# espnet/espnet

Hardware: AMD Instinct MI355X
Metric: audio-seconds/sec (RTF^-1), Conformer-ASR, 10 s utterances (higher is better)
Workload: dtype bf16; 1 GPU; BASELINE.json configs[1]: Conformer-small (12x256d, 4 heads), HIP STFT/log-mel + HIP encoder + greedy CTC (G1) + hypotheses collated to the host, 32 x 10 s utterances per GPU per step, V=5000; batch_per_gpu=32, global_batch=32, parallelism=utterance-dp1

## Files before the change

### espnet_amd/csrc/block.hip

```cpp
#include <stdio.h>
#include <stdlib.h>

#include <type_traits>

#include "em_common.h"
#include "switches.h"

namespace {

constexpr int D = 256;
constexpr int BM = 32;
constexpr int NT = 256;
constexpr int NC = 256;
constexpr int UNIT = 32768;
constexpr int PAR_FLOATS = EM_BLOCK_PARAM_GROUP;
constexpr int PAR_BYTES = PAR_FLOATS * 4;
constexpr int MAX_GROUPS = 4;
constexpr int PAR_OFF = 0;
constexpr int RED_OFF = PAR_OFF + MAX_GROUPS * PAR_BYTES;
constexpr int TOUCH_OFF = RED_OFF + 2048;
constexpr int TILE_OFF = TOUCH_OFF + 1024;
constexpr int ABUF_OFF = TILE_OFF + 32768;
constexpr int WK_OFF = ABUF_OFF + 16384;
constexpr int XCH_OFF = WK_OFF + 32768;
constexpr int XSLOT = 8192;
constexpr int SMEM_BYTES = XCH_OFF + 49152;
static_assert(ABUF_OFF % 1024 == 0 && TILE_OFF % 1024 == 0 && SMEM_BYTES <= 160 * 1024, "LDS layout");
constexpr int KW_MAX = 31, TROWS_MAX = BM + KW_MAX - 1;
constexpr int TPITCH = 528;
static_assert(TROWS_MAX * TPITCH <= 32768, "conv tile");
constexpr int CPAR_OFF = XCH_OFF;
constexpr int ABUF64_OFF = XCH_OFF + 8192;
static_assert(PAR_BYTES <= 8192 && ABUF64_OFF + 32768 <= SMEM_BYTES, "fold layout");

typedef const __attribute__((address_space(1))) unsigned char* GU8;
typedef const __attribute__((address_space(1))) bf16x8* GFRAG;
constexpr int BAR_UNIT = 1, BAR_PARAMS = 2, BAR_TILE = 4, BAR_LAST = 8;

#ifndef EM_BLOCK_DBG
#define EM_BLOCK_DBG 0
#endif

#ifndef EM_BLOCK_VAR
#define EM_BLOCK_VAR 0
#endif
#ifndef EM_BLOCK_FINE
#define EM_BLOCK_FINE 0
#endif

#define EM_LGKM0() asm volatile("s_waitcnt lgkmcnt(0)" ::: "memory")

__device__ __forceinline__ const unsigned char* em_uniform_ptr(const unsigned char* p) {
  const unsigned long long v = (unsigned long long)p;
  const unsigned lo = __builtin_amdgcn_readfirstlane((unsigned)v);
  const unsigned hi = __builtin_amdgcn_readfirstlane((unsigned)(v >> 32));
  return (const unsigned char*)(((unsigned long long)hi << 32) | lo);
}

template <int N, typename F>
__device__ __forceinline__ void em_static_for(F&& f) {
  if constexpr (N > 0) {
    em_static_for<N - 1>(f);
    f(std::integral_constant<int, N - 1>{});
  }
}

template <int MODE, int KWT = 31, bool RELU = false>
__global__ __launch_bounds__(NT, 1) void block_kernel(const EmBlockArgs a_in, long long* __restrict__ stamps) {
  const EmBlockArgs& a = a_in;
  const void *ffm_w1 = a_in.ffm_w1, *ffm_w2 = a_in.ffm_w2, *ff_w1 = a_in.ff_w1, *ff_w2 = a_in.ff_w2;
  const float *ffm_b1g = a_in.ffm_b1g, *ff_b1g = a_in.ff_b1g;
  int nsplit = 1;
  if constexpr (RELU && (MODE & (EM_BLOCK_A | EM_BLOCK_D | EM_BLOCK_T)) != 0) {
    nsplit = a_in.ffn_split > 1 ? a_in.ffn_split : 1;
    if (nsplit > 1) {
      const int nch_all = ((a_in.ff >> 6) + 1) & ~1, nch_s = nch_all / nsplit, sidx = blockIdx.z;
      const size_t wo = (size_t)sidx * nch_s * UNIT;
      if (ffm_w1) { ffm_w1 = (const unsigned char*)ffm_w1 + wo; ffm_w2 = (const unsigned char*)ffm_w2 + wo; }
      if (ff_w1) { ff_w1 = (const unsigned char*)ff_w1 + wo; ff_w2 = (const unsigned char*)ff_w2 + wo; }
      if (ffm_b1g) ffm_b1g += sidx * nch_s * 64;
      if (ff_b1g) ff_b1g += sidx * nch_s * 64;
    }
  }
  bool ffn_exit = false;
  constexpr int KW = KWT, HALF = KWT / 2, TROWS = BM + KWT - 1;
  static_assert(KWT == 31 || KWT == 15, "depthwise conv width");
  constexpr int dbg = EM_BLOCK_DBG;
  using MM = Mma<bf16>;
  constexpr bool HAS_C = (MODE & EM_BLOCK_C) != 0, HAS_D = (MODE & EM_BLOCK_D) != 0;
  constexpr bool HAS_A = (MODE & EM_BLOCK_A) != 0, FINAL = (MODE & EM_BLOCK_FINAL) != 0;
  constexpr bool CTC = (MODE & EM_BLOCK_CTC) != 0;
  constexpr bool FOLD = HAS_C && HAS_D;
  constexpr bool ATT = (MODE & EM_BLOCK_ATT) != 0;
  constexpr bool HAS_T = (MODE & EM_BLOCK_T) != 0, HAS_Q = (MODE & EM_BLOCK_Q) != 0;
  static_assert(!(HAS_T || HAS_Q) || (RELU && !HAS_C && !HAS_D && !HAS_A && !FINAL && !CTC && ATT == HAS_T), "block<ATT|T>, block<Q>, block<ATT|T|Q>");
  static_assert(!ATT || ((HAS_C != HAS_T) && !HAS_D && !HAS_A && !FINAL), "block<ATT|C> and block<ATT|T..> are the instantiations with the attention phase");
  static_assert(!FOLD || KWT == 31, "the folded C part is written for the 15-frame halo of k = 31");
  extern __shared__ __attribute__((aligned(1024))) unsigned char smem[];
  unsigned char* const abuf = smem + ABUF_OFF;
  float* const red0 = (float*)(smem + RED_OFF);
  float* const par = (float*)(smem + PAR_OFF);

  const int tid = threadIdx.x, lane = tid & 63;
  const int wave = __builtin_amdgcn_readfirstlane(tid >> 6);
  const int nf = wave & 3;
  const int lr = lane & 15, lg = lane >> 4;
  int b = blockIdx.y, t0 = blockIdx.x * BM;
  const int T = a.T;
  if constexpr (ATT) {
    const int gx = gridDim.x, lid = blockIdx.y * gx + blockIdx.x, grp = lid / (8 * gx);
    if ((int)blockIdx.y < a.B && grp * 8 + 8 <= a.B) {
      b = grp * 8 + (lid & 7);
      t0 = ((lid - grp * 8 * gx) >> 3) * BM;
    }
  }

  bool row_ok[2];
  size_t mrow[2];
#pragma unroll
  for (int mi = 0; mi < 2; ++mi) {
    const int t = t0 + mi * 16 + lr;
    row_ok[mi] = t < T;
    mrow[mi] = (size_t)b * T + (t < T ? t : T - 1);
  }
  const int ncol = nf * 16 + lg * 4;
  const int swz = lr & 7;
  const int tile_wr = lr * 128 + (((2 * nf + (lg >> 1)) ^ swz) << 4) + (lg & 1) * 8;
  const int nch = (((a.ff >> 6) + 1) & ~1) / nsplit;
  int nts = 0;
  auto stamp = [&](int code) __attribute__((always_inline)) {
    if constexpr (EM_BLOCK_FINE) {
      if (stamps && blockIdx.x == (gridDim.x > 3 ? 3 : 0) && blockIdx.y == (a.B > 5 ? 5 : 0) && blockIdx.z == 0 && lane == 0 && nts < 64)
        stamps[wave * 64 + nts] = ((long long)code << 56) | ((long long)__builtin_amdgcn_s_memtime() & 0xffffffffffffffll);
    } else {
      if (stamps && blockIdx.x == 0 && blockIdx.y == 0 && blockIdx.z < 4 && tid == 0 && nts < 64)
        stamps[blockIdx.z * 64 + nts] = ((long long)code << 56) | ((long long)__builtin_amdgcn_s_memtime() & 0xffffffffffffffll);
    }
    ++nts;
  };
  auto fstamp = [&](int code) __attribute__((always_inline)) {
    if constexpr (EM_BLOCK_FINE) stamp(code);
  };
  auto rstamp = [&](int code) __attribute__((always_inline)) {
    if constexpr (EM_BLOCK_FINE || RELU) stamp(code);
  };
  stamp(1);
  int nbar = 0;
  auto bar = [&](int code) __attribute__((always_inline)) {
    (void)code;
    ++nbar;
    EM_LGKM0();
    __builtin_amdgcn_s_barrier();
  };

  float4 xr[2][4];
  bf16x8 act[2][8];
  auto load_x = [&]() __attribute__((always_inline)) {
#pragma unroll
    for (int mi = 0; mi < 2; ++mi)
#pragma unroll
      for (int f = 0; f < 4; ++f) xr[mi][f] = *(const float4*)(a.x + mrow[mi] * D + 64 * f + ncol);
  };
  float* const xdst = FOLD ? a.x_out : a.x;
  auto store_x = [&]() __attribute__((always_inline)) {
#pragma unroll
    for (int mi = 0; mi < 2; ++mi)
      if (row_ok[mi]) {
#pragma unroll
        for (int f = 0; f < 4; ++f) *(float4*)(xdst + mrow[mi] * D + 64 * f + ncol) = xr[mi][f];
      }
  };
  constexpr bool PLAIN = !RELU && !FOLD;
  constexpr bool X_EARLY_A = PLAIN && HAS_A && !(EM_BLOCK_VAR & 0x10000);
  constexpr bool X_EARLY_C = PLAIN && HAS_C && !(EM_BLOCK_VAR & 0x20000);
  constexpr bool GLU_COUNTED = PLAIN && HAS_C && (EM_BLOCK_VAR & 0x40000) != 0;
  typedef __attribute__((ext_vector_type(2))) unsigned su32x2;
  typedef __attribute__((ext_vector_type(4))) unsigned su32x4;
  constexpr unsigned ROW_MASKED = 0x80000000u;
  unsigned rowoff[2];
#pragma unroll
  for (int mi = 0; mi < 2; ++mi) rowoff[mi] = row_ok[mi] ? (unsigned)(t0 + mi * 16 + lr) * (D * 4u) + ncol * 4u : ROW_MASKED;
  auto rows_rsrc = [&](const void* base, int esz) __attribute__((always_inline)) {
    const unsigned char* p = em_uniform_ptr((const unsigned char*)base + (size_t)b * T * D * esz);
    return __builtin_amdgcn_make_buffer_rsrc(const_cast<unsigned char*>(p), 0, T * D * esz, 0x00020000);
  };
  auto put_f32x4 = [&](__amdgpu_buffer_rsrc_t rs, int mi, int f, const float4& v) __attribute__((always_inline)) {
    __builtin_amdgcn_raw_buffer_store_b128(__builtin_bit_cast(su32x4, v), rs, rowoff[mi] + 256 * f, 0, 0);
  };
  auto put_bf16x4 = [&](__amdgpu_buffer_rsrc_t rs, int mi, int f, const bf16x4& v) __attribute__((always_inline)) {
    __builtin_amdgcn_raw_buffer_store_b64(__builtin_bit_cast(su32x2, v), rs, (rowoff[mi] >> 1) + 128 * f, 0, 0);
  };
  auto store_x_counted = [&]() __attribute__((always_inline)) {
    const __amdgpu_buffer_rsrc_t rs = rows_rsrc(xdst, 4);
#pragma unroll
    for (int mi = 0; mi < 2; ++mi)
#pragma unroll
      for (int f = 0; f < 4; ++f) put_f32x4(rs, mi, f, xr[mi][f]);
  };
  auto load_act = [&]() __attribute__((always_inline)) {
#pragma unroll
    for (int mi = 0; mi < 2; ++mi)
#pragma unroll
      for (int ks = 0; ks < 8; ++ks)
        act[mi][ks] = *(const bf16x8*)(abuf + ((ks >> 1) * 32 + mi * 16 + lr) * 128 + ((((ks & 1) * 4 + lg) ^ swz) << 4));
  };
  int nln = 0;
  auto ln_partials = [&](const float4 (&v)[2][4], float* red) {
#pragma unroll
    for (int mi = 0; mi < 2; ++mi) {
      float s = 0.f;
#pragma unroll
      for (int f = 0; f < 4; ++f) s += (v[mi][f].x + v[mi][f].y) + (v[mi][f].z + v[mi][f].w);
      const float m0 = s * (1.0f / 16.0f);
      float q = 0.f;
#pragma unroll
      for (int f = 0; f < 4; ++f) {
        const float dx = v[mi][f].x - m0, dy = v[mi][f].y - m0, dz = v[mi][f].z - m0, dw = v[mi][f].w - m0;
        q += (dx * dx + dy * dy) + (dz * dz + dw * dw);
      }
      {
        const Pair2 ps = wave_xor16_pair(s), pq = wave_xor16_pair(q);
        q = pq.a + pq.b + (ps.a - ps.b) * (ps.a - ps.b) * (1.0f / 32.0f);
        s = ps.a + ps.b;
      }
      {
        const Pair2 ps = wave_xor32_pair(s), pq = wave_xor32_pair(q);
        q = pq.a + pq.b + (ps.a - ps.b) * (ps.a - ps.b) * (1.0f / 64.0f);
        s = ps.a + ps.b;
      }
      red[nf * 32 + mi * 16 + lr] = s;
      red[128 + nf * 32 + mi * 16 + lr] = q;
    }
  };
  auto ln_finish = [&](const float* red, float mean[2], float rstd[2]) __attribute__((always_inline)) {
#pragma unroll
    for (int mi = 0; mi < 2; ++mi) {
      const int m = mi * 16 + lr;
      const float s0 = red[m], s1 = red[32 + m], s2 = red[64 + m], s3 = red[96 + m];
      const float q0 = red[128 + m], q1 = red[160 + m], q2 = red[192 + m], q3 = red[224 + m];
      const float sa = s0 + s1, sb = s2 + s3;
      const float qa = q0 + q1 + (s0 - s1) * (s0 - s1) * (1.0f / 128.0f);
      const float qb = q2 + q3 + (s2 - s3) * (s2 - s3) * (1.0f / 128.0f);
      const float qq = qa + qb + (sa - sb) * (sa - sb) * (1.0f / 256.0f);
      mean[mi] = (sa + sb) * (1.0f / D);
      const float var = qq * (1.0f / D) + a.eps;
      const float y0 = __builtin_amdgcn_rsqf(var);
      rstd[mi] = y0 * (1.5f - 0.5f * var * y0 * y0);
    }
  };
  auto no_pre = [] {};
  auto ln_stats = [&](float mean[2], float rstd[2], int code, auto&& pre1, auto n1c) __attribute__((always_inline)) {
    constexpr int N1 = decltype(n1c)::value;
    float* const red = red0 + (nln & 1) * 256;
    ++nln;
    pre1();
    ln_partials(xr, red);
    if constexpr (N1 > 0 && !(EM_BLOCK_VAR & 32)) {
#pragma unroll
      for (int i = 0; i < N1; ++i) {
        __builtin_amdgcn_sched_group_barrier(0x020, 1, 0);
        __builtin_amdgcn_sched_group_barrier(0x002, N1 > 16 ? 4 : 7, 0);
      }
    }
    fstamp(11);
    bar(code);
    fstamp(12);
    ln_finish(red, mean, rstd);
  };
  auto ln_apply_pre = [&](const float* pb, int go, int bo, float4 y[2][4], int code, auto&& pre1, auto n1c) __attribute__((always_inline)) {
    float mean[2], rstd[2];
    ln_stats(mean, rstd, code, pre1, n1c);
#pragma unroll
    for (int f = 0; f < 4; ++f) {
      const float4 g4 = *(const float4*)(pb + go + 64 * f + ncol);
      const float4 b4 = *(const float4*)(pb + bo + 64 * f + ncol);
#pragma unroll
      for (int mi = 0; mi < 2; ++mi) {
        y[mi][f].x = (xr[mi][f].x - mean[mi]) * rstd[mi] * g4.x + b4.x;
        y[mi][f].y = (xr[mi][f].y - mean[mi]) * rstd[mi] * g4.y + b4.y;
        y[mi][f].z = (xr[mi][f].z - mean[mi]) * rstd[mi] * g4.z + b4.z;
        y[mi][f].w = (xr[mi][f].w - mean[mi]) * rstd[mi] * g4.w + b4.w;
      }
    }
  };
  auto ln_apply = [&](const float* pb, int go, int bo, float4 y[2][4], int code) __attribute__((always_inline)) {
    ln_apply_pre(pb, go, bo, y, code, no_pre, std::integral_constant<int, 0>{});
  };
  auto ln_to_act_pre = [&](const float* pb, int go, int bo, int code, auto&& pre1, auto n1c, auto&& pre2, auto n2c) __attribute__((always_inline)) {
    constexpr int N2 = decltype(n2c)::value;
    float4 y[2][4];
    __builtin_amdgcn_sched_barrier(0);
    ln_apply_pre(pb, go, bo, y, 0, pre1, n1c);
    pre2();
#pragma unroll
    for (int mi = 0; mi < 2; ++mi)
#pragma unroll
      for (int f = 0; f < 4; ++f) {
        bf16x4 pk = {(bf16)y[mi][f].x, (bf16)y[mi][f].y, (bf16)y[mi][f].z, (bf16)y[mi][f].w};
        *(bf16x4*)(abuf + f * 4096 + mi * 2048 + tile_wr) = pk;
      }
    if constexpr (N2 > 0 && !(EM_BLOCK_VAR & 32)) {
#pragma unroll
      for (int i = 0; i < N2; ++i) {
        __builtin_amdgcn_sched_group_barrier(0x020, 1, 0);
        __builtin_amdgcn_sched_group_barrier(0x002, N2 > 8 ? 6 : 10, 0);
      }
    }
    fstamp(13);
    bar(code);
    fstamp(14);
    load_act();
  };
  auto ln_to_act = [&](const float* pb, int go, int bo, int code) __attribute__((always_inline)) {
    ln_to_act_pre(pb, go, bo, code, no_pre, std::integral_constant<int, 0>{}, no_pre, std::integral_constant<int, 0>{});
  };
  struct WF {
    bf16x8 v[8];
  };
  WF ring[4];
  const unsigned voff = nf * 8192 + lane * 16;
  auto read_unit = [&](const void* base, int u, WF& w) __attribute__((always_inline)) {
    GU8 su = (GU8)base + (size_t)u * UNIT + voff;
#pragma unroll
    for (int q = 0; q < 8; ++q) w.v[q] = *(GFRAG)(su + q * 1024);
  };
  auto k_pre = [&](const void* base, int n) __attribute__((always_inline)) {
#pragma unroll
    for (int j = 0; j < 3; ++j) read_unit(base, j < n ? j : n - 1, ring[j]);
  };
  auto stream_k = [&](const void* base, auto count, auto&& body) __attribute__((always_inline)) {
    constexpr int N = decltype(count)::value;
#pragma unroll
    for (int u = 0; u < N; ++u) {
      if (u + 3 < N) read_unit(base, u + 3, ring[(u + 3) & 3]);
      body(ring[u & 3], u);
    }
  };
  constexpr int MAXT = 16;
  auto touch = [&]() __attribute__((always_inline)) {
#ifdef EM_BLOCK_NO_TOUCH
    return;
#endif
    const int nwg = gridDim.x * gridDim.y;
    const int per_xcc = (nwg + 7) >> 3;
    const int nworker = per_xcc * 4;
    const int worker = (int)((blockIdx.y * gridDim.x + blockIdx.x) >> 3) * 4 + wave;
    const unsigned dst = TOUCH_OFF + wave * 256;
    const int loff = lane * 128;
    int total = (HAS_C ? 48 : 0) + (HAS_D ? 16 + 8 * nch : 0) + (HAS_A ? 48 + 8 * nch : 0) + (HAS_T ? 16 + 8 * nch : 0) +
                (HAS_Q ? 48 : 0);
    if (CTC) total += a.ctc_units * 4;
#pragma unroll 1
    for (int i = 0; i < MAXT && worker + i * nworker < total; ++i) {
      int j = worker + i * nworker;
      const unsigned char* p = nullptr;
      auto take = [&](const void* base, int n) __attribute__((always_inline)) {
        if (p == nullptr) {
          if (j < n) p = (const unsigned char*)base + (size_t)j * 8192;
          else j -= n;
        }
      };
      if (HAS_C) {
        take(a.wout, 16);
        take(a.pw1f, 32);
      }
      if (HAS_D) {
        take(a.pw2, 16);
        take(ff_w1, nch * 4);
        take(ff_w2, nch * 4);
      }
      if (HAS_A) {
        take(ffm_w1, nch * 4);
        take(ffm_w2, nch * 4);
        take(a.wqkv, 48);
      }
      if (HAS_T) {
        take(a.wout, 16);
        take(ff_w1, nch * 4);
        take(ff_w2, nch * 4);
      }
      if (HAS_Q) take(a.wqkv, 48);
      if (CTC) take(a.ctc_w, a.ctc_units * 4);
      unsigned keep;
      asm volatile(
          "s_mov_b32 %0, m0\n\t"
          "s_mov_b32 m0, %3\n\t"
          "s_nop 0\n\t"
          "global_load_lds_dword %1, %2\n\t"
          "s_mov_b32 m0, %0"
          : "=&s"(keep)
          : "v"(loff), "s"(p), "s"(dst)
          : "memory");
    }
  };
  auto touch_done = [&]() __attribute__((always_inline)) {};
  if ((int)blockIdx.y >= a.B) {
    touch();
    asm volatile("s_waitcnt vmcnt(0)" ::: "memory");
    return;
  }

  auto dma_lines = [&](const void* g, unsigned lds_off, auto n1k_c) __attribute__((always_inline)) {
    constexpr int n1k = decltype(n1k_c)::value;
    const unsigned voff16 = lane * 16;
#pragma unroll
    for (int i = 0; i < (n1k + 3) / 4; ++i) {
      int j = wave + 4 * i;
      j = j < n1k ? j : n1k - 1;
      const unsigned char* p = em_uniform_ptr((const unsigned char*)g + (size_t)j * 1024);
      const unsigned dst = __builtin_amdgcn_readfirstlane(lds_off + j * 1024);
      unsigned keep;
      asm volatile(
          "s_mov_b32 %0, m0\n\t"
          "s_mov_b32 m0, %3\n\t"
          "s_nop 0\n\t"
          "global_load_lds_dwordx4 %1, %2\n\t"
          "s_mov_b32 m0, %0"
          : "=&s"(keep)
          : "v"(voff16), "s"(p), "s"(dst)
          : "memory");
    }
  };

  auto mma_of = [&](const bf16x8 (&av)[2][8], const WF& w, bool swap, f32x4 out[2]) {
    if constexpr (dbg & 1) {
      out[0] = out[1] = (f32x4){0.f, 0.f, 0.f, 0.f};
      return;
    }
    f32x4 c[2][2];
#pragma unroll
    for (int mi = 0; mi < 2; ++mi) c[mi][0] = c[mi][1] = (f32x4){0.f, 0.f, 0.f, 0.f};
#pragma unroll
    for (int ks = 0; ks < 8; ++ks)
#pragma unroll
      for (int mi = 0; mi < 2; ++mi)
        c[mi][ks & 1] = swap ? MM::mma(av[mi][ks], w.v[ks], c[mi][ks & 1]) : MM::mma(w.v[ks], av[mi][ks], c[mi][ks & 1]);
    out[0] = c[0][0] + c[0][1];
    out[1] = c[1][0] + c[1][1];
  };
  auto mma_k = [&](const WF& w, bool swap, f32x4 out[2]) __attribute__((always_inline)) { mma_of(act, w, swap, out); };
  auto read_w2 = [&](const void* w2, int p, int half, WF& w) __attribute__((always_inline)) {
    GU8 su = (GU8)w2 + (size_t)p * (2 * UNIT) + nf * 16384 + half * 8192 + lane * 16;
#pragma unroll
    for (int q = 0; q < 8; ++q) w.v[q] = *(GFRAG)(su + q * 1024);
  };
  auto ffn_pre = [&](const void* w1, const void* w2) __attribute__((always_inline)) {
    read_unit(w1, 0, ring[0]);
    read_unit(w1, 1, ring[1]);
    read_w2(w2, 0, 0, ring[2]);
    read_w2(w2, 0, 1, ring[3]);
  };
  auto ffn = [&](const float* pb, int b1o, int b2o, float scale, const void* w1, const void* w2, bool repark,
                 const float* b1g, const void* nbase, auto&& after) __attribute__((always_inline)) {
    const int np = nch >> 1, lastc = nch - 1;
    auto read_w1 = [&](int c, WF& w) __attribute__((always_inline)) {
      const bool past = c >= nch;
      const void* b = (past && nbase) ? nbase : w1;
      const int u = past ? (nbase ? c - nch : lastc) : c;
      read_unit(b, u, w);
    };
    constexpr bool B1G = RELU;
    float4 nb0 = make_float4(0.f, 0.f, 0.f, 0.f), nb1 = nb0;
    if constexpr (B1G) {
      nb0 = *(const float4*)(b1g + ncol);
      nb1 = *(const float4*)(b1g + 64 + ncol);
    }
    auto act_ = [](float v) { return RELU ? fmaxf(v, 0.f) : swishf_(v); };
    f32x4 acc2[16][2];
#pragma unroll
    for (int f = 0; f < 16; ++f) acc2[f][0] = acc2[f][1] = (f32x4){0.f, 0.f, 0.f, 0.f};
    float4* const xpark = (float4*)(smem + TILE_OFF) + tid;
#pragma unroll
    for (int mi = 0; mi < 2; ++mi)
#pragma unroll
      for (int f = 0; f < 4; ++f) xpark[(mi * 4 + f) * NT] = xr[mi][f];
    auto swish_pack = [&](const f32x4 h[2][2], int p, bf16x8 hb[2]) __attribute__((always_inline)) {
      float4 b0, b1;
      if constexpr (B1G) {
        b0 = nb0;
        b1 = nb1;
        const int pn = p + 1 < np ? p + 1 : p;
        nb0 = *(const float4*)(b1g + (2 * pn) * 64 + ncol);
        nb1 = *(const float4*)(b1g + (2 * pn + 1) * 64 + ncol);
      } else {
        b0 = *(const float4*)(pb + b1o + (2 * p) * 64 + ncol);
        b1 = *(const float4*)(pb + b1o + (2 * p + 1) * 64 + ncol);
      }
#pragma unroll
      for (int mi = 0; mi < 2; ++mi)
        hb[mi] = (bf16x8){(bf16)act_(h[0][mi][0] + b0.x), (bf16)act_(h[0][mi][1] + b0.y),
                          (bf16)act_(h[0][mi][2] + b0.z), (bf16)act_(h[0][mi][3] + b0.w),
                          (bf16)act_(h[1][mi][0] + b1.x), (bf16)act_(h[1][mi][1] + b1.y),
                          (bf16)act_(h[1][mi][2] + b1.z), (bf16)act_(h[1][mi][3] + b1.w)};
    };
    auto mma_w2 = [&](const WF& w, int half, const bf16x8 hb[2]) __attribute__((always_inline)) {
      if constexpr (dbg & 1) return;
#pragma unroll
      for (int q = 0; q < 8; ++q) {
        acc2[half * 8 + q][0] = MM::mma(w.v[q], hb[0], acc2[half * 8 + q][0]);
        acc2[half * 8 + q][1] = MM::mma(w.v[q], hb[1], acc2[half * 8 + q][1]);
      }
    };
    f32x4 h[2][2];
    bf16x8 hb[2];
    mma_k(ring[0], false, h[0]);
    read_w1(2, ring[0]);
    mma_k(ring[1], false, h[1]);
    read_w1(3, ring[1]);
    swish_pack(h, 0, hb);
    bar(0);
    rstamp(20);
#pragma unroll 1
    for (int p = 0; p + 1 < np; ++p) {
      mma_k(ring[0], false, h[0]);
      read_w1(2 * p + 4, ring[0]);
      mma_k(ring[1], false, h[1]);
      read_w1(2 * p + 5, ring[1]);
      mma_w2(ring[2], 0, hb);
      read_w2(w2, p + 1, 0, ring[2]);
      mma_w2(ring[3], 1, hb);
      read_w2(w2, p + 1, 1, ring[3]);
      swish_pack(h, p + 1, hb);
    }
    mma_w2(ring[2], 0, hb);
    mma_w2(ring[3], 1, hb);
    after();
    rstamp(21);
    float4 psum[2][4];
    auto reduce_as = [&](auto nfc) __attribute__((always_inline)) {
      constexpr int NF = decltype(nfc)::value;
#pragma unroll
      for (int dst = 0; dst < 4; ++dst) {
        if (dst == NF) continue;
        unsigned char* slot = smem + ABUF_OFF + (dst * 3 + (NF > dst ? NF - 1 : NF)) * XSLOT + lane * 16;
#pragma unroll
        for (int f4 = 0; f4 < 4; ++f4)
#pragma unroll
          for (int mi = 0; mi < 2; ++mi) *(f32x4*)(slot + (f4 * 2 + mi) * 1024) = acc2[4 * f4 + dst][mi];
      }
      bar(0);
#pragma unroll
      for (int f4 = 0; f4 < 4; ++f4) {
        const float4 b4 = *(const float4*)(pb + b2o + 64 * f4 + ncol);
#pragma unroll
        for (int mi = 0; mi < 2; ++mi) {
          f32x4 sum;
          bool first = true;
#pragma unroll
          for (int src = 0; src < 4; ++src) {
            f32x4 v;
            if (src == NF) v = acc2[4 * f4 + NF][mi];
            else v = *(const f32x4*)(smem + ABUF_OFF + (NF * 3 + (src > NF ? src - 1 : src)) * XSLOT + lane * 16 + (f4 * 2 + mi) * 1024);
            sum = first ? v : sum + v;
            first = false;
          }
          if constexpr (RELU) {
            if (nsplit > 1) {
              psum[mi][f4] = make_float4(sum[0], sum[1], sum[2], sum[3]);
              continue;
            }
          }
          xr[mi][f4] = xpark[(mi * 4 + f4) * NT];
          xr[mi][f4].x += scale * (sum[0] + b4.x);
          xr[mi][f4].y += scale * (sum[1] + b4.y);
          xr[mi][f4].z += scale * (sum[2] + b4.z);
          xr[mi][f4].w += scale * (sum[3] + b4.w);
          if (repark) xpark[(mi * 4 + f4) * NT] = xr[mi][f4];
        }
      }
    };
    switch (nf) {
      case 0: reduce_as(std::integral_constant<int, 0>{}); break;
      case 1: reduce_as(std::integral_constant<int, 1>{}); break;
      case 2: reduce_as(std::integral_constant<int, 2>{}); break;
      default: reduce_as(std::integral_constant<int, 3>{}); break;
    }
    if constexpr (RELU) {
      if (nsplit > 1) {
        const int wg = b * (int)gridDim.x + (ATT ? t0 / BM : (int)blockIdx.x);
        float4* const part = (float4*)a.ffn_part + ((size_t)wg * nsplit) * 8 * NT;
        float4* const mine = part + (size_t)blockIdx.z * 8 * NT + tid;
        constexpr bool SEAM_ST_PLAIN = (EM_BLOCK_VAR & 8192) == 0, SEAM_LD_PLAIN = (EM_BLOCK_VAR & 4096) == 0;
        constexpr bool SEAM_REL = SEAM_ST_PLAIN, SEAM_ACQ = SEAM_LD_PLAIN;
        auto put = [&](float4* p, const float4& v) __attribute__((always_inline)) {
          if constexpr (SEAM_ST_PLAIN) {
            *p = v;
          } else {
            __hip_atomic_store((unsigned long long*)p, ((const unsigned long long*)&v)[0], __ATOMIC_RELAXED, __HIP_MEMORY_SCOPE_AGENT);
            __hip_atomic_store((unsigned long long*)p + 1, ((const unsigned long long*)&v)[1], __ATOMIC_RELAXED, __HIP_MEMORY_SCOPE_AGENT);
          }
        };
        auto get = [&](const float4* p) __attribute__((always_inline)) -> float4 {
          if constexpr (SEAM_LD_PLAIN) {
            return *p;
          } else {
            unsigned long long w[2];
            w[0] = __hip_atomic_load((const unsigned long long*)p, __ATOMIC_RELAXED, __HIP_MEMORY_SCOPE_AGENT);
            w[1] = __hip_atomic_load((const unsigned long long*)p + 1, __ATOMIC_RELAXED, __HIP_MEMORY_SCOPE_AGENT);
            float4 v;
            __builtin_memcpy(&v, w, 16);
            return v;
          }
        };
#pragma unroll
        for (int mi = 0; mi < 2; ++mi)
#pragma unroll
          for (int f4 = 0; f4 < 4; ++f4) put(mine + (mi * 4 + f4) * NT, psum[mi][f4]);
        asm volatile("s_waitcnt vmcnt(0)" ::: "memory");
        bar(0);
        int* const flag = (int*)(red0 + 480);
        if (tid == 0) {
          if constexpr (SEAM_REL) {
            __builtin_amdgcn_fence(__ATOMIC_RELEASE, "agent");
            asm volatile("s_waitcnt vmcnt(0)" ::: "memory");
          }
          const int t = __hip_atomic_fetch_add(a.ffn_ticket + wg, 1, __ATOMIC_RELAXED, __HIP_MEMORY_SCOPE_AGENT);
          if (t == nsplit - 1) {
            __hip_atomic_store(a.ffn_ticket + wg, 0, __ATOMIC_RELAXED, __HIP_MEMORY_SCOPE_AGENT);
            if constexpr (SEAM_ACQ) __builtin_amdgcn_fence(__ATOMIC_ACQUIRE, "agent");
          }
          *flag = t;
        }
        bar(0);
        if (*flag != nsplit - 1) {
          ffn_exit = true;
          return;
        }
        rstamp(23);
        auto sum_shares = [&](auto SC) __attribute__((always_inline)) {
          constexpr int SU = decltype(SC)::value;
#pragma unroll
          for (int mi = 0; mi < 2; ++mi) {
            float4 tot[4];
#pragma unroll
            for (int f4 = 0; f4 < 4; ++f4) tot[f4] = make_float4(0.f, 0.f, 0.f, 0.f);
            if constexpr (SU > 0) {
              float4 v[SU][4];
#pragma unroll
              for (int sp = 0; sp < SU; ++sp)
#pragma unroll
                for (int f4 = 0; f4 < 4; ++f4) v[sp][f4] = get(part + ((size_t)sp * 8 + (mi * 4 + f4)) * NT + tid);
#pragma unroll
              for (int sp = 0; sp < SU; ++sp)
#pragma unroll
                for (int f4 = 0; f4 < 4; ++f4) {
                  tot[f4].x += v[sp][f4].x; tot[f4].y += v[sp][f4].y; tot[f4].z += v[sp][f4].z; tot[f4].w += v[sp][f4].w;
                }
            } else {
              for (int sp = 0; sp < nsplit; ++sp)
#pragma unroll
                for (int f4 = 0; f4 < 4; ++f4) {
                  const float4 v = get(part + ((size_t)sp * 8 + (mi * 4 + f4)) * NT + tid);
                  tot[f4].x += v.x; tot[f4].y += v.y; tot[f4].z += v.z; tot[f4].w += v.w;
                }
            }
#pragma unroll
            for (int f4 = 0; f4 < 4; ++f4) {
              const float4 b4 = *(const float4*)(pb + b2o + 64 * f4 + ncol);
              xr[mi][f4] = xpark[(mi * 4 + f4) * NT];
              xr[mi][f4].x += scale * (tot[f4].x + b4.x);
              xr[mi][f4].y += scale * (tot[f4].y + b4.y);
              xr[mi][f4].z += scale * (tot[f4].z + b4.z);
              xr[mi][f4].w += scale * (tot[f4].w + b4.w);
              if (repark) xpark[(mi * 4 + f4) * NT] = xr[mi][f4];
            }
          }
        };
        if (nsplit == 2) sum_shares(std::integral_constant<int, 2>{});
        else if (nsplit == 4) sum_shares(std::integral_constant<int, 4>{});
        else sum_shares(std::integral_constant<int, 0>{});
        rstamp(24);
      }
    }
  };
  auto no_next = [](int) {};
  auto proj_resid = [&](const float* pb, int bo, const void* w, auto&& next) __attribute__((always_inline)) {
    stream_k(w, std::integral_constant<int, 4>{}, [&](const WF& cur, int f) {
      if (f > 0) next(f - 1);
      f32x4 c[2];
      mma_k(cur, false, c);
      const float4 b4 = *(const float4*)(pb + bo + 64 * f + ncol);
#pragma unroll
      for (int mi = 0; mi < 2; ++mi) {
        xr[mi][f].x += c[mi][0] + b4.x;
        xr[mi][f].y += c[mi][1] + b4.y;
        xr[mi][f].z += c[mi][2] + b4.z;
        xr[mi][f].w += c[mi][3] + b4.w;
      }
    });
    next(3);
  };

  constexpr int NG = (HAS_T || HAS_Q) ? (HAS_T && HAS_Q ? 2 : 1) : HAS_D ? (HAS_A ? 4 : 3) : (HAS_C ? 1 : 2);
  if constexpr (HAS_T && HAS_Q) {
    dma_lines(a.row0_src + (size_t)b * a.row_stride, PAR_OFF + 2 * PAR_BYTES, std::integral_constant<int, 1>{});
  }
  if (FOLD) {
    dma_lines(a.params_c, CPAR_OFF, std::integral_constant<int, PAR_BYTES / 1024>{});
  } else if (HAS_D) {
    dma_lines(a.dw_w, WK_OFF, std::integral_constant<int, KW>{});
    dma_lines(a.dw_b, WK_OFF + KW * 1024, std::integral_constant<int, 1>{});
  } else {
    dma_lines(a.params, PAR_OFF, std::integral_constant<int, NG * (PAR_BYTES / 1024)>{});
  }
  const float* const pb0 = par;
  const float* const pb1 = par + PAR_FLOATS;
  const float* const pb2 = par + 2 * PAR_FLOATS;
  const float* const pb3 = par + 3 * PAR_FLOATS;

  auto att_plain = [&]() __attribute__((always_inline)) {
    if constexpr (ATT && RELU) {
      typedef __attribute__((ext_vector_type(4))) unsigned u32x4;
      const int hh = wave;
      const int Tp = a.Tpad;
      const size_t bh = (size_t)b * 4 + hh;
      const bf16* const qb = (const bf16*)a.qh + bh * Tp * 64;
      const bf16* const kb = (const bf16*)a.kh + bh * Tp * 64;
      const bf16* const vb = (const bf16*)a.vt + bh * 64 * Tp;
      const int nkeys = a.att_mask ? T - 1 : T;
      bf16x8 qraw[2][2], kf[4][2];
      uint2 vraw[4][2][2];
#pragma unroll
      for (int mi = 0; mi < 2; ++mi)
#pragma unroll
        for (int ks = 0; ks < 2; ++ks) qraw[mi][ks] = *(const bf16x8*)(qb + (size_t)(t0 + 16 * mi + lr) * 64 + ks * 32 + lg * 8);
#pragma unroll
      for (int n = 0; n < 4; ++n)
#pragma unroll
        for (int ks = 0; ks < 2; ++ks) kf[n][ks] = *(const bf16x8*)(kb + (size_t)(16 * n + lr) * 64 + ks * 32 + lg * 8);
#pragma unroll
      for (int f = 0; f < 4; ++f)
#pragma unroll
        for (int jp = 0; jp < 2; ++jp)
#pragma unroll
          for (int hf = 0; hf < 2; ++hf)
            vraw[f][jp][hf] = *(const uint2*)(vb + (size_t)(16 * f + lr) * Tp + 32 * jp + 16 * hf + 4 * lg);
      read_unit(a.wout, 0, ring[0]);
      load_x();
      read_unit(a.wout, 1, ring[1]);
      read_unit(a.wout, 2, ring[2]);
      constexpr float LOG2E = 1.4426950408889634f;
      const bf16x8 ones = {(bf16)1.f, (bf16)1.f, (bf16)1.f, (bf16)1.f, (bf16)1.f, (bf16)1.f, (bf16)1.f, (bf16)1.f};
#pragma unroll
      for (int mi = 0; mi < 2; ++mi) {
        bf16x8 qf[2];
#pragma unroll
        for (int ks = 0; ks < 2; ++ks)
#pragma unroll
          for (int e = 0; e < 8; ++e) qf[ks][e] = (bf16)((float)qraw[mi][ks][e] * 0.125f);
        f32x4 sc[4];
#pragma unroll
        for (int n = 0; n < 4; ++n) sc[n] = (f32x4){0.f, 0.f, 0.f, 0.f};
#pragma unroll
        for (int ks = 0; ks < 2; ++ks)
#pragma unroll
          for (int n = 0; n < 4; ++n) sc[n] = MM::mma(kf[n][ks], qf[ks], sc[n]);
        float tm = -INFINITY;
#pragma unroll
        for (int n = 0; n < 4; ++n)
#pragma unroll
          for (int r = 0; r < 4; ++r) {
            sc[n][r] = (16 * n + 4 * lg + r) < nkeys ? sc[n][r] : -INFINITY;
            tm = fmaxf(tm, sc[n][r]);
          }
        tm = wave_xor16_max(tm);
        tm = wave_xor32_max(tm);
        const float mnl = tm * LOG2E;
        unsigned pbu[2][4];
#pragma unroll
        for (int n = 0; n < 4; ++n)
#pragma unroll
          for (int h2 = 0; h2 < 2; ++h2) {
            const float e0 = __builtin_amdgcn_exp2f(__builtin_fmaf(sc[n][2 * h2], LOG2E, -mnl));
            const float e1 = __builtin_amdgcn_exp2f(__builtin_fmaf(sc[n][2 * h2 + 1], LOG2E, -mnl));
            pbu[n >> 1][(n & 1) * 2 + h2] = __builtin_bit_cast(unsigned, __builtin_convertvector((f32x2){e0, e1}, bf16x2));
          }
        f32x4 acc_o[4], acc_l = (f32x4){0.f, 0.f, 0.f, 0.f};
#pragma unroll
        for (int f = 0; f < 4; ++f) acc_o[f] = (f32x4){0.f, 0.f, 0.f, 0.f};
#pragma unroll
        for (int jp = 0; jp < 2; ++jp) {
          const bf16x8 pbf = __builtin_bit_cast(bf16x8, (u32x4){pbu[jp][0], pbu[jp][1], pbu[jp][2], pbu[jp][3]});
          acc_l = MM::mma(ones, pbf, acc_l);
#pragma unroll
          for (int f = 0; f < 4; ++f) {
            unsigned w[4];
#pragma unroll
            for (int hf = 0; hf < 2; ++hf) {
              const int nv = nkeys - (32 * jp + 16 * hf + 4 * lg);
              w[2 * hf] = vraw[f][jp][hf].x & (nv >= 2 ? 0xffffffffu : (nv == 1 ? 0xffffu : 0u));
              w[2 * hf + 1] = vraw[f][jp][hf].y & (nv >= 4 ? 0xffffffffu : (nv == 3 ? 0xffffu : 0u));
            }
            acc_o[f] = MM::mma(__builtin_bit_cast(bf16x8, (u32x4){w[0], w[1], w[2], w[3]}), pbf, acc_o[f]);
          }
        }
        const bool none = a.att_mask && t0 + 16 * mi + lr == 0;
        const float inv = 1.0f / acc_l[0];
#pragma unroll
        for (int f = 0; f < 4; ++f) {
          const bf16x4 pk = {(bf16)(none ? 0.f : acc_o[f][0] * inv), (bf16)(none ? 0.f : acc_o[f][1] * inv),
                             (bf16)(none ? 0.f : acc_o[f][2] * inv), (bf16)(none ? 0.f : acc_o[f][3] * inv)};
          *(bf16x4*)(abuf + hh * 4096 + mi * 2048 + lr * 128 + (((2 * f + (lg >> 1)) ^ swz) << 4) + (lg & 1) * 8) = pk;
        }
      }
      asm volatile("s_waitcnt vmcnt(0)" ::: "memory");
      touch();
      bar(0);
      load_act();
      stamp(4);
    }
  };
  if (HAS_C && !HAS_D) {
    if constexpr (ATT && RELU) {
      att_plain();
    } else if constexpr (ATT) {
      typedef __attribute__((ext_vector_type(4))) float f4;
      typedef const __attribute__((address_space(1))) f4* GF4;
      constexpr int LDB = 84;
      const int hh = wave;
      int klen_raw;
      asm volatile("s_load_dword %0, %1, 0x0" : "=s"(klen_raw) : "s"(a.klens + b) : "memory");
      auto park_x = [&]() __attribute__((always_inline)) {
#pragma unroll
        for (int mi = 0; mi < 2; ++mi)
#pragma unroll
          for (int f = 0; f < 4; ++f) {
            const float* xp = a.x + mrow[mi] * D + 64 * f + ncol;
            const unsigned dst = __builtin_amdgcn_readfirstlane(TILE_OFF + ((mi * 4 + f) * NT + wave * 64) * 16);
            unsigned keep;
            asm volatile(
                "s_mov_b32 %0, m0\n\t"
                "s_mov_b32 m0, %2\n\t"
                "s_nop 0\n\t"
                "global_load_lds_dwordx4 %1, off\n\t"
                "s_mov_b32 m0, %0"
                : "=&s"(keep)
                : "v"(xp), "s"(dst)
                : "memory");
          }
      };
      const int Tp = a.Tpad;
      const size_t bh = (size_t)b * 4 + hh;
      GU8 qb = (GU8)a.qh + (bh * Tp + t0) * 128;
      const unsigned lo16 = lane * 16;
      GU8 kb = (GU8)em_uniform_ptr((const unsigned char*)a.kh + bh * Tp * 128);
      GU8 vb = (GU8)em_uniform_ptr((const unsigned char*)a.vt + bh * 64 * (size_t)Tp * 2);
      const int npg = a.ldp;
      const int g_q = 2 * (int)gridDim.x - (t0 >> 4);
      GU8 ppb = (GU8)em_uniform_ptr((const unsigned char*)a.pos + ((size_t)hh * npg + g_q) * 2048);
      struct KP {
        bf16x8 k[8], p[12];
      };
      struct VV {
        bf16x8 v[8];
      };
      auto load_kp = [&](int jt, KP& kp) __attribute__((always_inline)) {
        GU8 rk = kb + (size_t)jt * 8192;
#pragma unroll
        for (int i = 0; i < 8; ++i) kp.k[i] = *(GFRAG)(rk + i * 1024 + lo16);
        GU8 rp = ppb + (size_t)jt * 8192;
#pragma unroll
        for (int i = 0; i < 12; ++i) kp.p[i] = *(GFRAG)(rp + i * 1024 + lo16);
      };
      auto load_v = [&](int jt, VV& vv) __attribute__((always_inline)) {
        GU8 rv = vb + (size_t)jt * 8192;
#pragma unroll
        for (int i = 0; i < 8; ++i) vv.v[i] = *(GFRAG)(rv + i * 1024 + lo16);
      };
      bf16x8 qraw[2][2];
      f4 ur[2][2], vr[2][2];
#pragma unroll
      for (int mi = 0; mi < 2; ++mi)
#pragma unroll
        for (int ks = 0; ks < 2; ++ks) qraw[mi][ks] = *(GFRAG)(qb + (16 * mi + lr) * 128 + (ks * 4 + lg) * 16);
#pragma unroll
      for (int ks = 0; ks < 2; ++ks)
#pragma unroll
        for (int h2 = 0; h2 < 2; ++h2) {
          ur[ks][h2] = *(GF4)(a.pos_u + hh * 64 + ks * 32 + lg * 8 + h2 * 4);
          vr[ks][h2] = *(GF4)(a.pos_v + hh * 64 + ks * 32 + lg * 8 + h2 * 4);
        }
      KP kp;
      VV vv;
      load_kp(0, kp);
      load_v(0, vv);
      touch();
      int klen;
      {
        asm volatile("s_waitcnt lgkmcnt(0)" : "+s"(klen_raw) : : "memory");
        klen = klen_raw < T ? klen_raw : T;
        klen = klen > 0 ? klen : 1;
      }
      const int ntile = (klen + 63) >> 6, nfull = klen >> 6;
      bf16x8 qu[2][2], qv[2][2];
#pragma unroll
      for (int mi = 0; mi < 2; ++mi)
#pragma unroll
        for (int ks = 0; ks < 2; ++ks)
#pragma unroll
          for (int e = 0; e < 8; ++e) {
            const float qf = (float)qraw[mi][ks][e];
            qu[mi][ks][e] = (bf16)((qf + ur[ks][e >> 2][e & 3]) * 0.125f);
            qv[mi][ks][e] = (bf16)((qf + vr[ks][e >> 2][e & 3]) * 0.125f);
          }
      f32x4 acc_o[2][4], acc_l[2];
      float row_m[2] = {-INFINITY, -INFINITY};
#pragma unroll
      for (int mi = 0; mi < 2; ++mi) {
        acc_l[mi] = (f32x4){0.f, 0.f, 0.f, 0.f};
#pragma unroll
        for (int f = 0; f < 4; ++f) acc_o[mi][f] = (f32x4){0.f, 0.f, 0.f, 0.f};
      }
      const bf16x8 ones = {(bf16)1.f, (bf16)1.f, (bf16)1.f, (bf16)1.f, (bf16)1.f, (bf16)1.f, (bf16)1.f, (bf16)1.f};
      constexpr float LOG2E = 1.4426950408889634f;
      float* const bdw = (float*)(smem + XCH_OFF) + wave * (2 * 16 * LDB);
      const int last = ((klen + 63) >> 6) - 1;
      auto tile = [&](int jt, auto maskc) __attribute__((always_inline)) {
        constexpr bool MASK = decltype(maskc)::value;
        const int j0 = jt * 64;
        const int jn = jt < last ? jt + 1 : last;
        f32x4 sc[2][4], dd[2][5];
#pragma unroll
        for (int mi = 0; mi < 2; ++mi) {
#pragma unroll
          for (int n = 0; n < 4; ++n) sc[mi][n] = (f32x4){0.f, 0.f, 0.f, 0.f};
#pragma unroll
          for (int n = 0; n < 5; ++n) dd[mi][n] = (f32x4){0.f, 0.f, 0.f, 0.f};
        }
#pragma unroll
        for (int ks = 0; ks < 2; ++ks) {
#pragma unroll
          for (int pn = 0; pn < 6; ++pn) {
            if (pn >= 1) dd[0][pn - 1] = MM::mma(kp.p[2 * pn + ks], qv[0][ks], dd[0][pn - 1]);
            if (pn <= 4) dd[1][pn] = MM::mma(kp.p[2 * pn + ks], qv[1][ks], dd[1][pn]);
          }
        }
#pragma unroll
        for (int ks = 0; ks < 2; ++ks)
#pragma unroll
          for (int n = 0; n < 4; ++n)
#pragma unroll
            for (int mi = 0; mi < 2; ++mi) sc[mi][n] = MM::mma(kp.k[2 * n + ks], qu[mi][ks], sc[mi][n]);
        if constexpr (!(EM_BLOCK_VAR & 512)) load_kp(jn, kp);
        if (jt == last) park_x();
        if constexpr (!(EM_BLOCK_VAR & 256)) {
#pragma unroll
        for (int mi = 0; mi < 2; ++mi)
#pragma unroll
          for (int n = 0; n < 5; ++n)
            *(float4*)(bdw + (mi * 16 + lr) * LDB + 16 * n + 4 * lg) = make_float4(dd[mi][n][0], dd[mi][n][1], dd[mi][n][2], dd[mi][n][3]);
        }
        bf16x8 pb[2][2];
        float alpha[2];
#pragma unroll
        for (int mi = 0; mi < 2; ++mi) {
          const float* bdr = bdw + (mi * 16 + lr) * LDB + 15 - lr + 8 * lg;
#pragma unroll
          for (int n = 0; n < 4; ++n)
#pragma unroll
            for (int r = 0; r < 4; ++r) sc[mi][n][r] += (EM_BLOCK_VAR & 256) ? dd[mi][n][r] : bdr[32 * (n >> 1) + 4 * (n & 1) + r];
          if constexpr (MASK) {
            const int kl = klen - j0 - 8 * lg;
// ... 891 lines not shown
```

Baseline: 367,200 audio-s/s.

## Hand FFN hidden activations across waves through LDS instead of reducing partial outputs

In the fused FFN, each wave now writes its swish-activated hidden slice to a double-buffered LDS exchange area. Every wave reads all four slices and multiplies them against a w2 slice re-laid out by output column, so each wave owns complete output columns. This removes the end-of-FFN cross-wave partial-sum reduction through LDS and the parking of the residual in LDS. In exchange it adds one barrier per hidden-pair step and expects a different w2 weight layout.

```diff
diff --git a/espnet_amd/csrc/block.hip b/espnet_amd/csrc/block.hip
--- a/espnet_amd/csrc/block.hip
+++ b/espnet_amd/csrc/block.hip
@@ -23,9 +23,16 @@
 constexpr int ABUF_OFF = TILE_OFF + 32768;
 constexpr int WK_OFF = ABUF_OFF + 16384;
 constexpr int XCH_OFF = WK_OFF + 32768;
+#ifndef EM_BLOCK_VAR
+#define EM_BLOCK_VAR 0
+#endif
+constexpr bool FFN_HANDOVER = (EM_BLOCK_VAR & 0x80000) == 0;
+constexpr int HX_OFF = XCH_OFF;
+constexpr int HX_BUF = 8192, HX_SLICE = 2048;
 constexpr int XSLOT = 8192;
-constexpr int SMEM_BYTES = XCH_OFF + 49152;
+constexpr int SMEM_BYTES = XCH_OFF + (FFN_HANDOVER ? 45056 : 49152);
 static_assert(ABUF_OFF % 1024 == 0 && TILE_OFF % 1024 == 0 && SMEM_BYTES <= 160 * 1024, "LDS layout");
+static_assert(HX_OFF + 2 * HX_BUF <= SMEM_BYTES && XCH_OFF + 4 * (2 * 16 * 84) * 4 <= SMEM_BYTES, "hand-over slots, attention scratch");
 constexpr int KW_MAX = 31, TROWS_MAX = BM + KW_MAX - 1;
 constexpr int TPITCH = 528;
 static_assert(TROWS_MAX * TPITCH <= 32768, "conv tile");
@@ -41,9 +48,6 @@
 #define EM_BLOCK_DBG 0
 #endif
 
-#ifndef EM_BLOCK_VAR
-#define EM_BLOCK_VAR 0
-#endif
 #ifndef EM_BLOCK_FINE
 #define EM_BLOCK_FINE 0
 #endif
@@ -440,9 +444,15 @@
   };
   auto mma_k = [&](const WF& w, bool swap, f32x4 out[2]) __attribute__((always_inline)) { mma_of(act, w, swap, out); };
   auto read_w2 = [&](const void* w2, int p, int half, WF& w) __attribute__((always_inline)) {
-    GU8 su = (GU8)w2 + (size_t)p * (2 * UNIT) + nf * 16384 + half * 8192 + lane * 16;
-#pragma unroll
-    for (int q = 0; q < 8; ++q) w.v[q] = *(GFRAG)(su + q * 1024);
+    if constexpr (FFN_HANDOVER) {
+      GU8 su = (GU8)w2 + (size_t)p * (2 * UNIT) + half * 32768 + nf * 1024 + lane * 16;
+#pragma unroll
+      for (int q = 0; q < 8; ++q) w.v[q] = *(GFRAG)(su + (q >> 2) * 16384 + (q & 3) * 4096);
+    } else {
+      GU8 su = (GU8)w2 + (size_t)p * (2 * UNIT) + nf * 16384 + half * 8192 + lane * 16;
+#pragma unroll
+      for (int q = 0; q < 8; ++q) w.v[q] = *(GFRAG)(su + q * 1024);
+    }
   };
   auto ffn_pre = [&](const void* w1, const void* w2) __attribute__((always_inline)) {
     read_unit(w1, 0, ring[0]);
@@ -470,10 +480,13 @@
 #pragma unroll
     for (int f = 0; f < 16; ++f) acc2[f][0] = acc2[f][1] = (f32x4){0.f, 0.f, 0.f, 0.f};
     float4* const xpark = (float4*)(smem + TILE_OFF) + tid;
-#pragma unroll
-    for (int mi = 0; mi < 2; ++mi)
-#pragma unroll
-      for (int f = 0; f < 4; ++f) xpark[(mi * 4 + f) * NT] = xr[mi][f];
+    constexpr bool PARK = !FFN_HANDOVER;
+    if constexpr (PARK) {
+#pragma unroll
+      for (int mi = 0; mi < 2; ++mi)
+#pragma unroll
+        for (int f = 0; f < 4; ++f) xpark[(mi * 4 + f) * NT] = xr[mi][f];
+    }
     auto swish_pack = [&](const f32x4 h[2][2], int p, bf16x8 hb[2]) __attribute__((always_inline)) {
       float4 b0, b1;
       if constexpr (B1G) {
@@ -493,21 +506,61 @@
                           (bf16)act_(h[1][mi][0] + b1.x), (bf16)act_(h[1][mi][1] + b1.y),
                           (bf16)act_(h[1][mi][2] + b1.z), (bf16)act_(h[1][mi][3] + b1.w)};
     };
-    auto mma_w2 = [&](const WF& w, int half, const bf16x8 hb[2]) __attribute__((always_inline)) {
+    auto mma_w2 = [&](const WF& w, int half, const bf16x8 (*hv)[2]) __attribute__((always_inline)) {
       if constexpr (dbg & 1) return;
 #pragma unroll
       for (int q = 0; q < 8; ++q) {
-        acc2[half * 8 + q][0] = MM::mma(w.v[q], hb[0], acc2[half * 8 + q][0]);
-        acc2[half * 8 + q][1] = MM::mma(w.v[q], hb[1], acc2[half * 8 + q][1]);
-      }
+        const bf16x8* const b = FFN_HANDOVER ? hv[2 * half + (q >> 2)] : hv[0];
+        acc2[half * 8 + q][0] = MM::mma(w.v[q], b[0], acc2[half * 8 + q][0]);
+        acc2[half * 8 + q][1] = MM::mma(w.v[q], b[1], acc2[half * 8 + q][1]);
+      }
+    };
+    unsigned char* const hx = smem + HX_OFF + lane * 16;
+    auto hx_put = [&](int buf, const bf16x8 hb[2]) __attribute__((always_inline)) {
+#pragma unroll
+      for (int mi = 0; mi < 2; ++mi) *(bf16x8*)(hx + buf * HX_BUF + nf * HX_SLICE + mi * 1024) = hb[mi];
+    };
+    auto hx_get = [&](int buf, bf16x8 hv[4][2]) __attribute__((always_inline)) {
+#pragma unroll
+      for (int s = 0; s < 4; ++s)
+#pragma unroll
+        for (int mi = 0; mi < 2; ++mi) hv[s][mi] = *(const bf16x8*)(hx + buf * HX_BUF + s * HX_SLICE + mi * 1024);
     };
     f32x4 h[2][2];
-    bf16x8 hb[2];
+    bf16x8 hb[1][2];
     mma_k(ring[0], false, h[0]);
     read_w1(2, ring[0]);
     mma_k(ring[1], false, h[1]);
     read_w1(3, ring[1]);
-    swish_pack(h, 0, hb);
+    swish_pack(h, 0, hb[0]);
+    if constexpr (FFN_HANDOVER) {
+      bf16x8 hv[4][2];
+      auto meet = [&](int buf) __attribute__((always_inline)) {
+        __builtin_amdgcn_sched_barrier(0);
+        bar(0);
+        hx_get(buf, hv);
+        __builtin_amdgcn_sched_barrier(0);
+      };
+      hx_put(0, hb[0]);
+      rstamp(20);
+#pragma unroll 1
+      for (int p = 0; p + 1 < np; ++p) {
+        mma_k(ring[0], false, h[0]);
+        read_w1(2 * p + 4, ring[0]);
+        mma_k(ring[1], false, h[1]);
+        read_w1(2 * p + 5, ring[1]);
+        meet(p & 1);
+        mma_w2(ring[2], 0, hv);
+        read_w2(w2, p + 1, 0, ring[2]);
+        swish_pack(h, p + 1, hb[0]);
+        hx_put((p + 1) & 1, hb[0]);
+        mma_w2(ring[3], 1, hv);
+        read_w2(w2, p + 1, 1, ring[3]);
+      }
+      meet((np - 1) & 1);
+      mma_w2(ring[2], 0, hv);
+      mma_w2(ring[3], 1, hv);
+    } else {
     bar(0);
     rstamp(20);
 #pragma unroll 1
@@ -520,13 +573,37 @@
       read_w2(w2, p + 1, 0, ring[2]);
       mma_w2(ring[3], 1, hb);
       read_w2(w2, p + 1, 1, ring[3]);
-      swish_pack(h, p + 1, hb);
+      swish_pack(h, p + 1, hb[0]);
     }
     mma_w2(ring[2], 0, hb);
     mma_w2(ring[3], 1, hb);
+    }
     after();
     rstamp(21);
     float4 psum[2][4];
+    if constexpr (FFN_HANDOVER) {
+#pragma unroll
+      for (int f4 = 0; f4 < 4; ++f4) {
+        const float4 b4 = *(const float4*)(pb + b2o + 64 * f4 + ncol);
+#pragma unroll
+        for (int mi = 0; mi < 2; ++mi) {
+          f32x4 sum = acc2[f4][mi];
+#pragma unroll
+          for (int src = 1; src < 4; ++src) sum = sum + acc2[4 * src + f4][mi];
+          if constexpr (RELU) {
+            if (nsplit > 1) {
+              psum[mi][f4] = make_float4(sum[0], sum[1], sum[2], sum[3]);
+              continue;
+            }
+          }
+          xr[mi][f4].x += scale * (sum[0] + b4.x);
+          xr[mi][f4].y += scale * (sum[1] + b4.y);
+          xr[mi][f4].z += scale * (sum[2] + b4.z);
+          xr[mi][f4].w += scale * (sum[3] + b4.w);
+          if (repark) xpark[(mi * 4 + f4) * NT] = xr[mi][f4];
+        }
+      }
+    } else {
     auto reduce_as = [&](auto nfc) __attribute__((always_inline)) {
       constexpr int NF = decltype(nfc)::value;
 #pragma unroll
@@ -574,6 +651,7 @@
       case 1: reduce_as(std::integral_constant<int, 1>{}); break;
       case 2: reduce_as(std::integral_constant<int, 2>{}); break;
       default: reduce_as(std::integral_constant<int, 3>{}); break;
+    }
     }
     if constexpr (RELU) {
       if (nsplit > 1) {
@@ -657,7 +735,7 @@
 #pragma unroll
             for (int f4 = 0; f4 < 4; ++f4) {
               const float4 b4 = *(const float4*)(pb + b2o + 64 * f4 + ncol);
-              xr[mi][f4] = xpark[(mi * 4 + f4) * NT];
+              if constexpr (PARK) xr[mi][f4] = xpark[(mi * 4 + f4) * NT];
               xr[mi][f4].x += scale * (tot[f4].x + b4.x);
               xr[mi][f4].y += scale * (tot[f4].y + b4.y);
               xr[mi][f4].z += scale * (tot[f4].z + b4.z);
```

Measured after the change: 374,000 audio-s/s (median of 6 runs). 1.9% higher.
